# aous72/OpenJPH

Hardware: AMD Instinct MI355X
Metric: Msamples/s encode+decode, 8K 12-bit 4:4:4; achieved HBM GB/s vs roofline (higher is better)
Workload: dtype f32; 1 GPU; c3_8k_444_12b_irv97; width=7680, height=4320, components=3, bit_depth=12, wavelet=9/7 irreversible, decomps=5, hip_streams=1, sample_container_bits=16, roundtrip_max_abs_err=8

## Files before the change

openjph_amd/csrc/kernels_ht_enc.hip:

```cpp
#include <hip/hip_runtime.h>
#include <stdint.h>
#include <cstdlib>
#include <type_traits>
#include "../../include/ojphgpu.h"
#include "ht_quant.h"
#include "ht_tables.h"

namespace ojphgpu {
__device__ __attribute__((aligned(16))) uint16_t g_enc_vlc[2][2048];
}

namespace {

using ojphgpu::to_sign_mag;

constexpr int MS_WORDS = 512;
constexpr int VLC_WORDS = 64;
constexpr int MEL_CAP = 192;
constexpr int VLC_CAP = 3072 - MEL_CAP;
constexpr int WAVES = 4;
constexpr uint32_t NARROW_MAX_W = 64;

constexpr int MS_WORDS64 = 1040;
constexpr int VLC_WORDS64 = 96;
// ... 198 lines not shown
    for (int i = 0; i < 6; ++i) {
      V t = (active && !first_row) ? sample(x0 - 1 + i, y0 - 1) : (V)0;
      V v = ((V)(t + t) >> p) & ~(V)1;
      Eab[i] = expo(v); Sab[i] = v != 0;
    }

    uint32_t rho[2], cq[2], uq[2], Uq[2], tup[2];
    V msv[8]; uint32_t msl[8];
    uint32_t rho_q[2] = { 0, 0 }, emax[2] = { 0, 0 }, e[8];
#pragma unroll
    for (int i = 0; i < 8; ++i) {
      e[i] = expo(val[i]);
      if (val[i]) rho_q[i >> 2] |= 1u << (i & 3);
      emax[i >> 2] = max(emax[i >> 2], e[i]);
    }
    if (!has_q1) { rho_q[1] = 0; emax[1] = 0; }
    uint32_t rho_prev = __shfl_up(rho_q[1], 1);
    if (lane == 0) rho_prev = carry_rho;
    if (px == 0) rho_prev = 0;
    carry_rho = rdlane(rho_q[1], 63);
#pragma unroll
    for (int q = 0; q < 2; ++q) {
      const uint32_t rl = q == 0 ? rho_prev : rho_q[0];
      uint32_t kappa = 1, c;
      if (first_row) c = (rl >> 1) | (rl & 1);
      else {
        const uint32_t* E = Eab + 2 * q; const uint32_t* S = Sab + 2 * q;
        uint32_t me = max(max(E[0], E[1]), max(E[2], E[3]));
        int max_e = (int)me - 1;
        if (rho_q[q] & (rho_q[q] - 1)) kappa = (uint32_t)max(1, max_e);
        c = (S[0] | S[1]) | ((S[2] | S[3]) << 2) | ((rl & 4) >> 1) | ((rl & 8) >> 2);
      }
      const uint32_t U = max(emax[q], kappa), u = U - kappa;
      uint32_t eps = 0;
      if (u > 0) {
#pragma unroll
        for (int nn = 0; nn < 4; ++nn) eps |= (uint32_t)(e[q * 4 + nn] == emax[q]) << nn;
      }
      const uint32_t tuple = s_vlc[first_row ? 0 : 1][(c << 8) + (rho_q[q] << 4) + eps];
      rho[q] = rho_q[q]; cq[q] = c; uq[q] = u; Uq[q] = U; tup[q] = tuple;
#pragma unroll
      for (int nn = 0; nn < 4; ++nn) {
        const int i = q * 4 + nn;
        const uint32_t m = ((rho_q[q] >> nn) & 1u) ? U - ((tuple >> nn) & 1u) : 0u;
        const V s = val[i] ? val[i] - 2u + sgn[i] : (V)0;
        msl[i] = m;
        msv[i] = m ? (s & ((m >= VBITS ? (V)0 : ((V)1 << m)) - (V)1)) : (V)0;
      }
    }
    const bool q0on = active, q1on = has_q1;
    if (!q1on) { uq[1] = 0; for (int nn = 4; nn < 8; ++nn) { msl[nn] = 0; msv[nn] = 0; } }
    if (!q0on) { uq[0] = 0; for (int nn = 0; nn < 4; ++nn) { msl[nn] = 0; msv[nn] = 0; } }
    any_sig |= (__ballot(((rho[0] | rho[1]) != 0 && active) || over != 0u) != 0ull) ? 1u : 0u;

    uint64_t vb = 0; uint32_t vl = 0;
    auto vadd = [&](uint32_t c, uint32_t len) { vb |= (uint64_t)c << vl; vl += len; };
    uint32_t x0e = 0, xl0 = 0, x1e = 0, xl1 = 0;
    auto uvlc = [](uint32_t u, uint32_t& pre, uint32_t& pl, uint32_t& suf, uint32_t& sl, uint32_t& ext, uint32_t& el) {
      ext = 0; el = 0;
      if (u == 0) { pre = 0; pl = 0; suf = 0; sl = 0; }
      else if (u == 1) { pre = 1; pl = 1; suf = 0; sl = 0; }
      else if (u == 2) { pre = 2; pl = 2; suf = 0; sl = 0; }
      else if (u <= 4) { pre = 4; pl = 3; suf = u - 3; sl = 1; }
      else if (u <= 32 || !S64) { pre = 0; pl = 3; suf = u - 5; sl = 5; }
      else { pre = 0; pl = 3; suf = 28u + ((u - 33u) & 3u); sl = 5; ext = (u - 33u) >> 2; el = 4; }
    };
    bool ev2_valid = false; uint32_t ev2_bit = 0;
    if (q0on) {
      vadd(tup[0] >> 8, (tup[0] >> 4) & 7);
      if (q1on) vadd(tup[1] >> 8, (tup[1] >> 4) & 7);
      const uint32_t u0 = uq[0], u1 = uq[1];
      uint32_t p0, l0, s0, sl0, p1, l1, s1, sl1;
      if (first_row && u0 > 0 && u1 > 0) { ev2_valid = true; ev2_bit = min(u0, u1) > 2; }
      if (first_row && u0 > 2 && u1 > 2) {
        uvlc(u0 - 2, p0, l0, s0, sl0, x0e, xl0); uvlc(u1 - 2, p1, l1, s1, sl1, x1e, xl1);
        vadd(p0, l0); vadd(p1, l1); vadd(s0, sl0); vadd(s1, sl1); vadd(x0e, xl0); vadd(x1e, xl1);
      } else if (first_row && u0 > 2 && u1 > 0) {
        uvlc(u0, p0, l0, s0, sl0, x0e, xl0);
        vadd(p0, l0); vadd(u1 - 1, 1); vadd(s0, sl0); vadd(x0e, xl0);
      } else {
        uvlc(u0, p0, l0, s0, sl0, x0e, xl0); uvlc(u1, p1, l1, s1, sl1, x1e, xl1);
        vadd(p0, l0); vadd(p1, l1); vadd(s0, sl0); vadd(s1, sl1); vadd(x0e, xl0); vadd(x1e, xl1);
      }
    }

    const bool ev0_valid = q0on && cq[0] == 0, ev1_valid = q1on && cq[1] == 0;
    const uint32_t ev0_bit = rho[0] != 0, ev1_bit = rho[1] != 0;
    {
      const uint32_t cnt = (uint32_t)ev0_valid + (uint32_t)ev1_valid + (uint32_t)ev2_valid;
      const uint32_t incl = wave_incl_scan(cnt, lane);
      const uint32_t nev = rdlane(incl, 63);
      uint32_t at = incl - cnt;
      if (ev0_valid) { if (ev0_bit) atomicOr(&L.ev[at >> 5], 1u << (at & 31)); at++; }
      if (ev1_valid) { if (ev1_bit) atomicOr(&L.ev[at >> 5], 1u << (at & 31)); at++; }
      if (ev2_valid) { if (ev2_bit) atomicOr(&L.ev[at >> 5], 1u << (at & 31)); at++; }
      wave_sync();
      uint32_t done = 0;
      while (done < nev) {
        const uint32_t w = done >> 5, sh = done & 31;
        uint32_t word = rdfirst(L.ev[w]) >> sh;
        const uint32_t avail = min(32u - sh, nev - done);
        if (word == 0) { mel_zero_run(mel, L.mel, avail, lane); done += avail; continue; }
        const uint32_t z = (uint32_t)__builtin_ctz(word);
        if (z >= avail) { mel_zero_run(mel, L.mel, avail, lane); done += avail; continue; }
        mel_zero_run(mel, L.mel, z, lane);
        mel_one(mel, L.mel, lane);
        done += z + 1;
      }
      wave_sync();
      if (lane < 8) L.ev[lane] = 0;
    }

    {
      uint32_t tot = 0;
#pragma unroll
      for (int i = 0; i < 8; ++i) tot += msl[i];
      const uint32_t incl = wave_incl_scan(tot, lane);
      const uint32_t T = ms_carry + rdlane(incl, 63);
      uint32_t at = ms_carry + incl - tot;
#pragma unroll
      for (int i = 0; i < 8; ++i) {
        if constexpr (S64) {
          const uint32_t lo = msl[i] < 32u ? msl[i] : 32u;
          or_bits(L.ms, at, (uint32_t)msv[i], lo);
          if (msl[i] > 32u) or_bits(L.ms, at + 32u, (uint32_t)(msv[i] >> 32), msl[i] - 32u);
        } else or_bits(L.ms, at, (uint32_t)msv[i], msl[i]);
        at += msl[i];
      }
      wave_sync();
      uint32_t pos = 0;
      for (;;) {
        const uint32_t first_n = ms_ff ? 7u : 8u;
        const uint32_t start = pos + (lane == 0 ? 0u : first_n + 8u * (uint32_t)(lane - 1));
        const uint32_t nb = lane == 0 ? first_n : 8u;
        const bool ok = start + nb <= T;
        const uint32_t v = ok ? get_bits(L.ms, start, nb) : 0u;
        const uint64_t m_ok = __ballot(ok), m_ff = __ballot(ok && v == 0xFF);
        const uint32_t n_ok = m_ok == ~0ull ? 64u : (uint32_t)__builtin_ctzll(~m_ok);
        const uint32_t f_ff = m_ff ? (uint32_t)__builtin_ctzll(m_ff) : 64u;
        const uint32_t nc = min(n_ok, f_ff + 1u);
        if (nc == 0) break;
        if (ms_k + nc > ms_cap) { err = 1; break; }
        if ((uint32_t)lane < nc) ms_out[ms_k + lane] = (uint8_t)v;
        ms_k += nc;
        pos += first_n + 8u * (nc - 1u);
        ms_ff = f_ff < n_ok ? 1u : 0u;
      }
      const uint32_t rem = T - pos;
      const uint32_t cv = rem ? get_bits(L.ms, pos, rem) : 0u;
      wave_sync();
      const uint32_t used = (T >> 5) + 2;
      for (uint32_t i = lane; i < used && i < (uint32_t)MSW; i += 64) L.ms[i] = 0;
      wave_sync();
      if (lane == 0) L.ms[0] = cv;
      ms_carry = rem;
      wave_sync();
    }

    {
      const uint32_t incl = wave_incl_scan(vl, lane);
      const uint32_t T = v_carry + rdlane(incl, 63);
      {
        const uint32_t at = v_carry + incl - vl, lo = vl < 32u ? vl : 32u;
        or_bits(L.vlc, at, (uint32_t)vb, lo);
        if (vl > 32u) or_bits(L.vlc, at + 32u, (uint32_t)(vb >> 32), vl - 32u);
      }
      wave_sync();
      uint32_t pos = 0;
      for (;;) {
        const uint32_t start = pos + 8u * (uint32_t)lane;
        const bool have7 = start + 7 <= T, have8 = start + 8 <= T;
        const uint32_t v8 = have7 ? get_bits(L.vlc, start, 8) : 0u;
        uint32_t pv = __shfl_up(v8, 1);
        if (lane == 0) pv = v_prev;
        const bool special = have7 && pv > 0x8F && (v8 & 0x7F) == 0x7F;
        const bool stop = !have8 && !special;
        const uint64_t m_sp = __ballot(special), m_st = __ballot(stop);
        const uint32_t fs = m_sp ? (uint32_t)__builtin_ctzll(m_sp) : 64u;
        const uint32_t ft = m_st ? (uint32_t)__builtin_ctzll(m_st) : 64u;
        const uint32_t n8 = min(fs, ft);
        const bool sp = fs < ft;
        if (n8 == 0 && !sp) break;
        if (v_pos + n8 + 1 >= (uint32_t)VLC_CAP) { err = 1; break; }
        if ((uint32_t)lane < n8) *(vlc_last - (v_pos + lane)) = (uint8_t)v8;
        if (sp && (uint32_t)lane == fs) *(vlc_last - (v_pos + lane)) = 0x7F;
        const uint32_t last8 = n8 ? rdlane(v8, (int)(n8 - 1)) : v_prev;
        v_pos += n8 + (sp ? 1u : 0u);
        pos += 8u * n8 + (sp ? 7u : 0u);
        v_prev = sp ? 0x7Fu : last8;
      }
      const uint32_t rem = T - pos;
      const uint32_t cv = rem ? get_bits(L.vlc, pos, rem) : 0u;
      wave_sync();
      for (int i = lane; i < VLW; i += 64) L.vlc[i] = 0;
      wave_sync();
      if (lane == 0) L.vlc[0] = cv;
      v_carry = rem;
      wave_sync();
    }
    if (err) break;
  }

  err |= mel.err;
  uint32_t total = 0, ms_len = ms_k;
  if (!err && any_sig) {
    const uint32_t ms_tmp0 = rdfirst(L.ms[0]);
    if (ms_carry) {
      const uint32_t maxb = ms_ff ? 7u : 8u, t = maxb - ms_carry;
      const uint32_t tmp = ms_tmp0 | ((0xFFu & ((1u << t) - 1u)) << ms_carry);
      if (tmp != 0xFF) {
        if (ms_len >= ms_cap) err = 1;
        else { if (lane == 0) ms_out[ms_len] = (uint8_t)tmp; ms_len++; }
      }
    } else if (ms_ff) ms_len--;
    if (mel.run > 0) mel_put(mel, L.mel, 1, 1, lane);
    const uint32_t need = mel.lastff ? 7u : 8u, remaining = need - mel.nb;
    const uint32_t mel_tmp = (mel.acc << remaining) & 0xFFu;
    const uint32_t mel_mask = (0xFFu << remaining) & 0xFFu;
    const uint32_t vlc_tmp = rdfirst(L.vlc[0]) & 0xFFu;
    const uint32_t vlc_mask = v_carry ? (0xFFu >> (8 - v_carry)) : 0u;
    if ((mel_mask | vlc_mask) != 0) {
      if (mel.pos >= (uint32_t)MEL_CAP) err = 1;
      else {
        const uint32_t fuse = mel_tmp | vlc_tmp;
        if (((((fuse ^ mel_tmp) & mel_mask) | ((fuse ^ vlc_tmp) & vlc_mask)) == 0) && fuse != 0xFF && v_pos > 1) {
          if (lane == 0) L.mel[mel.pos] = (uint8_t)fuse;
          mel.pos++;
        } else {
          if (v_pos >= (uint32_t)VLC_CAP) err = 1;
          else {
            if (lane == 0) { L.mel[mel.pos] = (uint8_t)mel_tmp; *(vlc_last - v_pos) = (uint8_t)vlc_tmp; }
            mel.pos++; v_pos++;
          }
        }
      }
    }
    err |= mel.err;
    total = ms_len + mel.pos + v_pos;
  }
  wave_sync();
  __threadfence_block();

  uint32_t off = 0;
  if (err) total = 0;
  if (total) {
    off = claim_output(cursor, regions, nreg, bi, (total + 3u) & ~3u, out_cap, lane);
    if (off == 0xFFFFFFFFu) { err = 1; total = 0; off = 0; }
  }
  if (total) {
    const uint32_t scup = mel.pos + v_pos;
    uint8_t* dst = out + off;
    const uint8_t* vsrc = vlc_last - v_pos + 1;
    for (uint32_t i = lane; i < total; i += 64) {
      uint32_t b;
      if (i < ms_len) b = ms_out[i];
      else if (i < ms_len + mel.pos) b = L.mel[i - ms_len];
      else b = vsrc[i - ms_len - mel.pos];
      if (i == total - 1) b = scup >> 4;
      else if (i == total - 2) b = (b & 0xF0u) | (scup & 0xFu);
      dst[i] = (uint8_t)b;
    }
  }
  if (lane == 0) {
    results[bi].offset = off; results[bi].length = total;
    if (err) atomicOr(status, 1u);
  }
}

#ifndef ABL
#define ABL 0
#endif
#ifndef NWAVES
#define NWAVES 4
#endif
#ifndef NOUT_CAP
#define NOUT_CAP 5120
#endif
#ifndef NWAVES_PER_EU
#define NWAVES_PER_EU 4
#endif
constexpr uint32_t OUT_CAP = NOUT_CAP;
constexpr int PMS_WORDS = 576;
constexpr int PVLC_WORDS = 112;

struct NarrowLds {
  uint32_t out[OUT_CAP / 4];
  uint32_t ms[PMS_WORDS];
  uint32_t vlc[PVLC_WORDS];
  uint8_t  mel[MEL_CAP + 8];
};
static_assert(MEL_CAP + 8 >= 4 * (MEL_CAP / 4 + 2), "raw MEL words");
#ifndef NWG_PER_CU
#define NWG_PER_CU 4
#endif
static_assert(NWG_PER_CU * (2 * 2048 * 2 + 64 * 4 + NWAVES * sizeof(NarrowLds)) <= 160 * 1024, "the narrow kernel's workgroups do not fit the LDS as planned");

#ifndef ENC_ROWS_W4V
#define ENC_ROWS_W4V 1
#endif
#ifndef ENC_ROWS_AHEAD
#define ENC_ROWS_AHEAD 1
#endif
static_assert(ENC_ROWS_AHEAD == 1 || ENC_ROWS_AHEAD == 2, "one or two steps of rows in flight");

struct __attribute__((aligned(4))) U4 { uint32_t x, y, z, w; };
typedef uint32_t U4V __attribute__((ext_vector_type(4), aligned(4)));

template <int KIND> struct RawRows {
  uint32_t t[4], b[4];
  __device__ __forceinline__ void arrived() { asm volatile("" : "+v"(t[0]), "+v"(t[1]), "+v"(t[2]), "+v"(t[3]), "+v"(b[0]), "+v"(b[1]), "+v"(b[2]), "+v"(b[3])); }
  __device__ __forceinline__ uint32_t top(int k) const { return t[k]; }
  __device__ __forceinline__ uint32_t bot(int k) const { return b[k]; }
};
template <> struct RawRows<1> {
  U4V t, b;
  __device__ __forceinline__ void arrived() { asm volatile("" : "+v"(t), "+v"(b)); }
  __device__ __forceinline__ uint32_t top(int k) const { return t[k]; }
  __device__ __forceinline__ uint32_t bot(int k) const { return b[k]; }
};

__device__ __forceinline__ uint32_t dpp_prev(uint32_t v) { return (uint32_t)__builtin_amdgcn_update_dpp(0, (int)v, 0x138, 0xF, 0xF, false); }
__device__ __forceinline__ uint32_t dpp_next(uint32_t v) { return (uint32_t)__builtin_amdgcn_update_dpp(0, (int)v, 0x130, 0xF, 0xF, false); }

__device__ __forceinline__ uint32_t uvlc_word(uint32_t u)
{
  const uint32_t lo = u < 3u ? 1u : 0u, mid = (u >= 3u && u < 5u) ? 1u : 0u;
  const uint32_t pre = lo ? u : (mid ? 4u : 0u);
  const uint32_t pl = u < 3u ? u : 3u;
  const uint32_t suf = lo ? 0u : (mid ? u - 3u : u - 5u);
  const uint32_t sl = lo ? 0u : (mid ? 1u : 5u);
  return pre | (pl << 8) | (suf << 16) | (sl << 24);
}

constexpr uint64_t MEL_PM = (1ull << 0) | (1ull << 1) | (1ull << 2) | (1ull << 3) | (1ull << 5) | (1ull << 7) | (1ull << 9) | (1ull << 13) |
                            (1ull << 17) | (1ull << 21) | (1ull << 29) | (1ull << 37) | (1ull << 53);
constexpr uint32_t MEL_RAW_BITS = 8u * MEL_CAP;
constexpr uint32_t MEL_RAW_WORDS = MEL_CAP / 4 + 2;

__device__ __forceinline__ void mel_at(uint32_t k, uint32_t c, uint32_t& K, uint32_t& run, uint32_t& ones, uint32_t& pKm1)
{
  const uint32_t full = c >= 85u ? (c - 53u) >> 5 : 0u;
  const uint32_t cc = c - 32u * full;
  if (cc >= 53u) { K = 12u; run = cc - 53u; pKm1 = 37u; }
  else {
    const uint64_t m = MEL_PM << (63u - cc);
    const uint32_t lz = (uint32_t)__builtin_clzll(m);
    K = (uint32_t)__popcll(m) - 1u; run = lz;
    const uint64_t m2 = m & ~(0x8000000000000000ull >> lz);
    pKm1 = m2 ? cc - (uint32_t)__builtin_clzll(m2) : 0u;
  }
  ones = K - k + full;
}

__device__ __forceinline__ void mel_stuff(const uint32_t* raw, uint32_t total_bits, uint8_t* out, MelState& st, int lane)
{
  uint32_t pos = 0, bytes = 0, lastff = 0, err = 0;
  for (;;) {
    const uint32_t first = lastff ? 7u : 8u;
    const uint32_t start = pos + (lane == 0 ? 0u : first + 8u * ((uint32_t)lane - 1u));
    const uint32_t len = lane == 0 ? first : 8u;
    const bool have = start + len <= total_bits;
    const uint32_t w = start >> 5, sh = start & 31u;
    const uint32_t x = have ? __funnelshift_l(raw[w + 1], raw[w], sh) >> (32u - len) : 0u;
    const uint64_t m_have = __ballot(have), m_ff = __ballot(have && x == 0xFFu);
    const uint32_t n_ok = m_have == ~0ull ? 64u : (uint32_t)__builtin_ctzll(~m_have);
    const uint32_t f_ff = m_ff ? (uint32_t)__builtin_ctzll(m_ff) : 64u;
    const uint32_t nc = min(n_ok, f_ff + 1u);
    if (nc == 0) break;
    if (bytes + nc > (uint32_t)MEL_CAP) { err = 1; break; }
    if ((uint32_t)lane < nc) out[bytes + lane] = (uint8_t)x;
    bytes += nc;
    pos += first + 8u * (nc - 1u);
    lastff = f_ff < n_ok ? 1u : 0u;
  }
  const uint32_t left = total_bits - pos;
  const uint32_t w = pos >> 5, sh = pos & 31u;
  const uint32_t x = left ? rdfirst(__funnelshift_l(raw[w + 1], raw[w], sh)) >> (32u - left) : 0u;
  st.k = 0; st.run = 0; st.acc = x; st.nb = left; st.pos = bytes; st.lastff = lastff; st.err = err;
}

template <bool REV, int LOGP>
__global__ __launch_bounds__(64 * NWAVES) __attribute__((amdgpu_waves_per_eu(NWAVES_PER_EU, 8))) void ht_encode_kernel(
    const ojphgpu_cb_desc* __restrict__ blocks, uint32_t n, const uint32_t* __restrict__ coef,
    uint8_t* __restrict__ scratch, uint8_t* __restrict__ out, uint32_t out_cap,
    ojphgpu_cb_result* __restrict__ results, uint32_t* __restrict__ cursor, uint32_t* __restrict__ status,
    const uint32_t* __restrict__ regions, uint32_t nreg)
{
  __shared__ __attribute__((aligned(16))) uint16_t s_vlc[2][2048];
  __shared__ uint32_t s_uvlc[64];
  __shared__ NarrowLds s_wave[NWAVES];
  const int lane = threadIdx.x & 63;
  const int wave = __builtin_amdgcn_readfirstlane((int)(threadIdx.x >> 6));
  const uint32_t bi = blockIdx.x * NWAVES + wave;
  struct DescWords { uint32_t v[sizeof(ojphgpu_cb_desc) / 4]; } dw;
  __builtin_memcpy(&dw, blocks + min(bi, n - 1u), sizeof dw);
  ojphgpu_cb_desc d;
  __builtin_memcpy(&d, &dw, sizeof d);
  static_assert(offsetof(ojphgpu_cb_desc, K_max) == 16 && offsetof(ojphgpu_cb_desc, reversible) == 17, "K_max, reversible: bytes 0, 1 of dword 4");
  uint32_t kr = dw.v[4];
  asm volatile("" : "+s"(kr));
  const uint32_t d_K_max = kr & 0xFFu, d_reversible = (kr >> 8) & 0xFFu;
  const uint32_t W = d.w, H = d.h;
  constexpr uint32_t PPR = 1u << LOGP, RPS = 64u >> LOGP;
  const bool my_width = LOGP == 5 ? (W > NARROW_MAX_W && W <= 4u * PPR) : (W <= NARROW_MAX_W && W <= 4u * PPR);
  const bool my_kind = bi < n && my_width && ((d_reversible & 1u) != 0) == REV && (d_reversible & 4u) == 0;
  const bool mine = my_kind && W != 0 && H != 0;
  NarrowLds& L = s_wave[wave];
  uint8_t* outb = reinterpret_cast<uint8_t*>(L.out);
  const uint32_t K = d_K_max, p = 31u - K;
  constexpr bool rev = REV;
  const float delta_inv = rev ? 0.0f : __fdiv_rn(1.0f, d.delta);
  const uint32_t* src = coef + d.coef_off;
  const uint32_t pitch = d.pitch;
  uint8_t* ms_spill = scratch + d.data_off;
  const uint32_t ms_cap = d.scratch_cap > (uint32_t)VLC_CAP ? d.scratch_cap - VLC_CAP : 0;
  const uint32_t QW = (W + 1) >> 1, QH = (H + 1) >> 1, PW = (QW + 1) >> 1;
  const uint32_t nsteps = (QH + RPS - 1u) / RPS;

  const uint32_t r = (uint32_t)lane >> LOGP, px = (uint32_t)lane & (PPR - 1u);
  const bool pxok = px < PW;
  const uint32_t x0 = 4u * px;
  const bool has_q1 = pxok && x0 + 2 < W;

  auto prologue = [&](bool clear) __attribute__((always_inline)) {
    for (int i = threadIdx.x; i < 2 * 2048 / 8; i += blockDim.x)
      reinterpret_cast<uint4*>(&s_vlc[0][0])[i] = reinterpret_cast<const uint4*>(&ojphgpu::g_enc_vlc[0][0])[i];
    if (threadIdx.x < 64) s_uvlc[threadIdx.x] = uvlc_word(threadIdx.x);
    if (clear) {
      for (int i = lane; i < PMS_WORDS; i += 64) L.ms[i] = 0;
      for (int i = lane; i < PVLC_WORDS; i += 64) L.vlc[i] = 0;
      if (lane < (int)MEL_RAW_WORDS) reinterpret_cast<uint32_t*>(L.mel)[lane] = 0;
      wave_sync();
      if (lane == 0) { L.vlc[0] = 0xF; outb[OUT_CAP - 1] = 0xFF; }
      wave_sync();
    }
    __syncthreads();
  };
  if (!mine) {
    prologue(false);
    if (my_kind && lane == 0) { results[bi].offset = 0; results[bi].length = 0; }
    return;
  }
  const bool w4 = (W & 3u) == 0;

  uint32_t ms_pend = 0, ms_base = 0, ms_k = 0, ms_ff = 0;
  uint32_t v_pend = 4, v_base = 0, v_pos = 1, v_prev = 0xFF;
  uint32_t mel_k = 0, mel_c = 0, mel_bits = 0, mel_err = 0;
  uint32_t* const mel_raw = reinterpret_cast<uint32_t*>(L.mel);
  auto mel_or = [&](uint32_t code, uint32_t len, uint32_t pos) __attribute__((always_inline)) {
    if (len) {
      const uint32_t sh = pos & 31u, w = pos >> 5;
      const uint64_t v = (uint64_t)code << (64u - sh - len);
      atomicOr(&mel_raw[w], (uint32_t)(v >> 32));
      if (sh + len > 32u) atomicOr(&mel_raw[w + 1u], (uint32_t)v);
    }
  };
  auto mel_ones = [&](uint32_t n) __attribute__((always_inline)) {
    if (n == 0u) return;
    if (mel_bits + n > MEL_RAW_BITS) mel_err = 1;
    else if (lane == 0) mel_or((1u << n) - 1u, n, mel_bits);
    mel_bits += n;
  };
  auto mel_zeros = [&](uint32_t n) __attribute__((always_inline)) {
    mel_c += n;
    if (mel_c >= 85u) {
      const uint32_t full = (mel_c - 53u) >> 5;
      mel_ones(12u - mel_k + full);
      mel_k = 12u; mel_c -= 32u * full;
    }
  };
  uint32_t err = 0, any_sig = 0;
  bool prev_sig = false;

  uint32_t ms_out = 0;
  auto flush_stage = [&]() __attribute__((always_inline)) -> bool {
    const uint32_t have = ms_k - ms_out, nwd = have >> 2;
    if (ms_out + 4u * nwd > ms_cap) return false;
    uint32_t* g = reinterpret_cast<uint32_t*>(ms_spill + ms_out);
    for (uint32_t i = lane; i < nwd; i += 64) g[i] = L.out[i];
    const uint32_t keep = L.out[nwd];
    wave_sync();
    if (lane == 0) L.out[0] = keep;
    wave_sync();
    ms_out += 4u * nwd;
    return true;
  };

  uint32_t last_S = 0;

  auto ms_windows = [&](uint32_t base, uint32_t T, bool flush) __attribute__((always_inline)) -> uint32_t {
    uint32_t pos = base;
    for (;;) {
      const uint32_t first_n = ms_ff ? 7u : 8u;
      if (!flush && pos + first_n + 8u * 255u > T) break;
      const uint32_t start = pos + (lane == 0 ? 0u : first_n + 8u * (4u * (uint32_t)lane - 1u));
      const uint32_t lead = lane == 0 ? first_n : 8u;
      uint32_t v = 0, cnt = 0;
      if (start + lead <= T) {
        const uint32_t w = start >> 5, sh = start & 31u;
        v = __funnelshift_r(L.ms[w], L.ms[w + 1], sh);
        cnt = min(4u, 1u + ((T - start - lead) >> 3));
      }
      const uint32_t bytes = (lane == 0 && first_n == 7u) ? ((v & 0x7Fu) | ((v >> 7) << 8)) : v;
      const uint32_t have = cnt == 4u ? 0xFFFFFFFFu : (1u << (8u * cnt)) - 1u;
      const uint32_t ffm = (((bytes & 0x7F7F7F7Fu) + 0x01010101u) & bytes & 0x80808080u) & have;
      const uint64_t m_full = __ballot(cnt == 4u), m_ff = __ballot(ffm != 0u);
      const uint32_t nfull = m_full == ~0ull ? 64u : (uint32_t)__builtin_ctzll(~m_full);
      const uint32_t n_ok = nfull == 64u ? 256u : 4u * nfull + rdlane(cnt, (int)nfull);
      uint32_t f_ff = 256u;
      if (m_ff) { const uint32_t lf = (uint32_t)__builtin_ctzll(m_ff); f_ff = 4u * lf + ((uint32_t)__builtin_ctz(rdlane(ffm, (int)lf)) >> 3); }
      const uint32_t nc = min(n_ok, f_ff + 1u);
      if (nc == 0) break;
      if (ms_k - ms_out + nc + v_pos + 72u > OUT_CAP && !flush_stage()) { err = 1; break; }
      uint8_t* dstb = outb + (ms_k - ms_out) + 4u * (uint32_t)lane;
      const uint32_t mine = nc > 4u * (uint32_t)lane ? min(4u, nc - 4u * (uint32_t)lane) : 0u;
      if (mine > 0) dstb[0] = (uint8_t)bytes;
      if (mine > 1) dstb[1] = (uint8_t)(bytes >> 8);
      if (mine > 2) dstb[2] = (uint8_t)(bytes >> 16);
      if (mine > 3) dstb[3] = (uint8_t)(bytes >> 24);
      ms_k += nc;
      pos += first_n + 8u * (nc - 1u);
      ms_ff = f_ff < n_ok ? 1u : 0u;
    }
    return pos;
  };
  auto ms_windows_full = [&](uint32_t base, uint32_t T) __attribute__((always_inline)) -> uint32_t {
    uint32_t pos = base;
    for (;;) {
      const uint32_t first_n = ms_ff ? 7u : 8u;
      if (pos + first_n + 8u * 255u > T) break;
      const uint32_t start = lane == 0 ? pos : pos + first_n - 8u + 32u * (uint32_t)lane;
      const uint32_t w = start >> 5, sh = start & 31u;
      uint32_t bytes = __funnelshift_r(L.ms[w], L.ms[w + 1], sh);
      if (ms_ff) bytes = lane == 0 ? ((bytes & 0x7Fu) | ((bytes >> 7) << 8)) : bytes;
      const uint32_t ffm = ((bytes & 0x7F7F7F7Fu) + 0x01010101u) & bytes & 0x80808080u;
      const uint64_t m_ff = __ballot(ffm != 0u);
      uint32_t nc = 256u, ff = 0u;
      if (m_ff) { const uint32_t lf = (uint32_t)__builtin_ctzll(m_ff); nc = 4u * lf + ((uint32_t)__builtin_ctz(rdlane(ffm, (int)lf)) >> 3) + 1u; ff = 1u; }
      if (ms_k - ms_out + nc + v_pos + 72u > OUT_CAP && !flush_stage()) { err = 1; break; }
      if (4u * (uint32_t)lane < nc) __builtin_memcpy(outb + (ms_k - ms_out) + 4u * (uint32_t)lane, &bytes, 4);
      ms_k += nc;
      pos += first_n + 8u * (nc - 1u);
      ms_ff = ff;
    }
    return pos;
  };
  auto vlc_windows_full = [&](uint32_t base, uint32_t T) __attribute__((always_inline)) -> uint32_t {
    uint32_t pos = base;
    for (;;) {
      if (pos + 8u * 64u > T) break;
      const uint32_t v8 = get_bits(L.vlc, pos + 8u * (uint32_t)lane, 8);
      uint32_t pv = dpp_prev(v8);
      if (lane == 0) pv = v_prev;
      const uint64_t m_sp = __ballot(pv > 0x8Fu && (v8 & 0x7Fu) == 0x7Fu);
      uint32_t n8 = 64u, sp = 0u;
      if (m_sp) { n8 = (uint32_t)__builtin_ctzll(m_sp); sp = 1u; }
      if (v_pos + n8 + 1 >= (uint32_t)VLC_CAP) { err = 1; break; }
      if (ms_k - ms_out + v_pos + n8 + 72u > OUT_CAP && !flush_stage()) { err = 1; break; }
      if ((uint32_t)lane < n8 + sp) outb[OUT_CAP - 1 - (v_pos + lane)] = (uint8_t)((uint32_t)lane == n8 ? 0x7Fu : v8);
      const uint32_t last8 = n8 ? rdlane(v8, (int)(n8 - 1)) : v_prev;
      v_pos += n8 + sp;
      pos += 8u * n8 + 7u * sp;
      v_prev = sp ? 0x7Fu : last8;
    }
    return pos;
  };
  auto vlc_windows = [&](uint32_t base, uint32_t T, bool flush) __attribute__((always_inline)) -> uint32_t {
    uint32_t pos = base;
    for (;;) {
      if (!flush && pos + 8u * 64u > T) break;
      const uint32_t start = pos + 8u * (uint32_t)lane;
      const bool have7 = start + 7 <= T, have8 = start + 8 <= T;
      const uint32_t v8 = have7 ? get_bits(L.vlc, start, 8) : 0u;
      uint32_t pv = dpp_prev(v8);
      if (lane == 0) pv = v_prev;
      const bool special = have7 && pv > 0x8F && (v8 & 0x7F) == 0x7F;
      const bool stop = !have8 && !special;
      const uint64_t m_sp = __ballot(special), m_st = __ballot(stop);
      const uint32_t fs = m_sp ? (uint32_t)__builtin_ctzll(m_sp) : 64u;
      const uint32_t ft = m_st ? (uint32_t)__builtin_ctzll(m_st) : 64u;
      const uint32_t n8 = min(fs, ft);
      const bool sp = fs < ft;
      if (n8 == 0 && !sp) break;
      if (v_pos + n8 + 1 >= (uint32_t)VLC_CAP) { err = 1; break; }
      if (ms_k - ms_out + v_pos + n8 + 72u > OUT_CAP && !flush_stage()) { err = 1; break; }
      if ((uint32_t)lane < n8) outb[OUT_CAP - 1 - (v_pos + lane)] = (uint8_t)v8;
      if (sp && (uint32_t)lane == fs) outb[OUT_CAP - 1 - (v_pos + lane)] = 0x7F;
      const uint32_t last8 = n8 ? rdlane(v8, (int)(n8 - 1)) : v_prev;
      v_pos += n8 + (sp ? 1u : 0u);
      pos += 8u * n8 + (sp ? 7u : 0u);
      v_prev = sp ? 0x7Fu : last8;
    }
    return pos;
  };
  auto compact = [&](uint32_t* buf, uint32_t pos, uint32_t T, uint32_t nwords) __attribute__((always_inline)) -> uint32_t {
    const uint32_t rem = T - pos, nw = (rem + 31u) >> 5;
    const uint32_t w0 = pos >> 5, sh = pos & 31u;
    uint32_t keep = 0;
    if ((uint32_t)lane < nw) {
      keep = __funnelshift_r(buf[w0 + lane], buf[w0 + lane + 1], sh);
      if (lane == (int)nw - 1 && (rem & 31u)) keep &= (1u << (rem & 31u)) - 1u;
    }
    wave_sync();
    const uint32_t used = min((T >> 5) + 2u, nwords);
    for (uint32_t i = lane; i < used; i += 64) buf[i] = 0;
    wave_sync();
    if ((uint32_t)lane < nw) buf[lane] = keep;
    wave_sync();
    return rem;
  };

  auto or32 = [&](uint32_t* buf, uint32_t pos, uint32_t v) __attribute__((always_inline)) {
    const uint32_t sh = pos & 31u;
    uint32_t* wp = buf + (pos >> 5);
    atomicOr(wp, v << sh);
    atomicOr(wp + 1, (v >> 1) >> (sh ^ 31u));
  };
  auto nz_flags = [](uint32_t x) __attribute__((always_inline)) -> uint32_t { return (x + 0x7F7F7F7Fu) & 0x80808080u; };
  auto gather4 = [](uint32_t f) __attribute__((always_inline)) -> uint32_t { return ((f >> 7) * 0x10204080u) >> 28; };
  typedef unsigned short us2 __attribute__((ext_vector_type(2)));
  auto pk_max = [](uint32_t a, uint32_t b2) __attribute__((always_inline)) -> uint32_t {
    return __builtin_bit_cast(uint32_t, __builtin_elementwise_max(__builtin_bit_cast(us2, a), __builtin_bit_cast(us2, b2)));
  };
  auto left_of = [&](uint32_t v) __attribute__((always_inline)) -> uint32_t {
    if (LOGP == 4) return (uint32_t)__builtin_amdgcn_update_dpp(0, (int)v, 0x111, 0xF, 0xF, false);
    const uint32_t t = dpp_prev(v); return px == 0 ? 0u : t;
  };
  auto right_of = [&](uint32_t v) __attribute__((always_inline)) -> uint32_t {
    if (LOGP == 4) return (uint32_t)__builtin_amdgcn_update_dpp(0, (int)v, 0x101, 0xF, 0xF, false);
    const uint32_t t = dpp_next(v); return px == PPR - 1u ? 0u : t;
  };

  auto code_steps = [&](auto kind_c) __attribute__((always_inline)) {
    constexpr int KIND = decltype(kind_c)::value;
    using Rows = RawRows<KIND>;
    auto load_rows = [&](uint32_t qy, Rows& R) __attribute__((always_inline)) {
      const uint32_t qyc = min(qy, QH - 1u);
      const uint32_t y0 = 2u * qyc, y1 = min(y0 + 1u, H - 1u);
      const uint32_t* r0 = src + (size_t)y0 * pitch;
      const uint32_t* r1 = src + (size_t)y1 * pitch;
      if (ABL & 32) { r0 = coef + (size_t)bi * 4096u + y0 * 64u; r1 = coef + (size_t)bi * 4096u + y1 * 64u; }
      if constexpr (KIND == 1) {
        const uint32_t xc = min(x0, W - 4u);
        R.t = *reinterpret_cast<const U4V*>(r0 + xc);
        R.b = *reinterpret_cast<const U4V*>(r1 + xc);
      } else if (KIND == 0 && w4) {
        const uint32_t xc = min(x0, W - 4u);
        const U4 a = *reinterpret_cast<const U4*>(r0 + xc);
        const U4 c = *reinterpret_cast<const U4*>(r1 + xc);
        R.t[0] = a.x; R.t[1] = a.y; R.t[2] = a.z; R.t[3] = a.w;
        R.b[0] = c.x; R.b[1] = c.y; R.b[2] = c.z; R.b[3] = c.w;
      } else {
#pragma unroll
        for (int k = 0; k < 4; ++k) { const uint32_t xk = min(x0 + (uint32_t)k, W - 1u); R.t[k] = r0[xk]; R.b[k] = r1[xk]; }
      }
    };
    Rows A;
    [[maybe_unused]] Rows B;
    load_rows(r, A);
    if constexpr (ENC_ROWS_AHEAD == 2) load_rows(r + RPS, B);
    prologue(true);

    float colf[4]; uint32_t colm[4];
#pragma unroll
    for (int k = 0; k < 4; ++k) {
      const bool in = pxok && x0 + (uint32_t)k < W;
      colf[k] = in ? ldexpf(delta_inv, -(int)p) : 0.0f;
      colm[k] = in ? (1u << (31u - p)) - 1u : 0u;
    }
    const bool ragged = (QH & (RPS - 1u)) != 0 || (H & 1u) != 0;

    auto one_step = [&](const uint32_t step, Rows& R) __attribute__((always_inline)) {
      const uint32_t qy = RPS * step + r;
      const bool active = pxok && qy < QH;
      R.arrived();
      uint32_t rt[4], rb[4];
#pragma unroll
      for (int k = 0; k < 4; ++k) { rt[k] = R.top(k); rb[k] = R.bot(k); }
      if (ragged && step + 1 == nsteps) {
        const bool bot = active && 2u * qy + 1u < H;
#pragma unroll
        for (int k = 0; k < 4; ++k) { rt[k] = active ? rt[k] : 0u; rb[k] = bot ? rb[k] : 0u; }
      }
      uint32_t mu[8], sx[8];
      uint32_t nz = 0;
#pragma unroll
      for (int k = 0; k < 4; ++k) {
#pragma unroll
        for (int j = 0; j < 2; ++j) {
          const uint32_t raw = j ? rb[k] : rt[k];
          if (rev) {
            const int v = (int)raw;
            const uint32_t a = (uint32_t)(v >= 0 ? v : -v);
            mu[2 * k + j] = a & colm[k];
            sx[2 * k + j] = raw | (a << p);
            nz |= a;
          } else {
            mu[2 * k + j] = (uint32_t)__fmul_rn(fabsf(__uint_as_float(raw)), colf[k]);
            sx[2 * k + j] = raw;
            nz |= mu[2 * k + j];
          }
        }
      }
      if (__ballot((nz >> K) != 0u) != 0ull) {
        any_sig |= (rev ? __ballot(((nz >> K) & 1u) != 0u) != 0ull : true) ? 1u : 0u;
        if (!rev) {
          nz = 0;
#pragma unroll
          for (int i = 0; i < 8; ++i) { mu[i] = (mu[i] >> K) ? 0u : mu[i]; nz |= mu[i]; }
        }
      }
      if (rev) nz &= (1u << K) - 1u;
      if (ENC_ROWS_AHEAD == 2 || step + 1 < nsteps) load_rows(qy + ENC_ROWS_AHEAD * RPS, R);
      if (ENC_ROWS_AHEAD == 2 && err) return;
      if (ABL & 16) { any_sig |= (uint32_t)(__ballot((mu[0] ^ mu[1] ^ mu[2] ^ mu[3] ^ mu[4] ^ mu[5] ^ mu[6] ^ mu[7]) == 0x12345u) != 0ull); return; }
      {
        const bool step_sig = __ballot(nz != 0u) != 0ull;
        const bool skip = !step_sig && !prev_sig;
        prev_sig = step_sig;
        if (skip) {
          const uint32_t nq = (uint32_t)__popcll(__ballot(active)) + (uint32_t)__popcll(__ballot(has_q1 && active));
          mel_zeros(nq);
          last_S = 0;
          return;
        }
        any_sig |= step_sig ? 1u : 0u;
      }
      uint32_t e[8], sv[8];
#pragma unroll
      for (int i = 0; i < 8; ++i) {
        const uint32_t m1 = mu[i] - 1u, w = m1 + mu[i];
        e[i] = (0u - (uint32_t)__builtin_clz(w)) & 31u;
        sv[i] = __builtin_amdgcn_alignbit(m1, sx[i], 31);
      }
      const uint32_t ep0 = e[0] | (e[1] << 8) | (e[2] << 16) | (e[3] << 24);
      const uint32_t ep1 = e[4] | (e[5] << 8) | (e[6] << 16) | (e[7] << 24);
      const uint32_t sf0 = nz_flags(ep0), sf1 = nz_flags(ep1);
      const uint32_t rho0 = gather4(sf0), rho1 = gather4(sf1);
      const uint32_t emax0 = max(max(e[0], e[1]), max(e[2], e[3])), emax1 = max(max(e[4], e[5]), max(e[6], e[7]));

      uint32_t S;
      {
        const uint32_t b0 = e[1], b1 = e[3], b2 = e[5], b3 = e[7];
        const uint32_t m12 = max(b1, b2);
        const uint32_t own = max(b0, m12) | (max(m12, b3) << 16);
        const uint32_t X = b3 | (b0 << 16), Y = b0 | (b3 << 16);
        const uint32_t nb = (left_of(X) & 0xFFFFu) | (right_of(X) & 0xFFFF0000u);
        const uint32_t mx = pk_max(own, nb);
        const uint32_t F = (pk_max(nb, Y) + 0x007F001Fu) & 0x00800020u;
        const uint32_t f12 = ((m12 + 31u) & 32u) * 0x10004u;
        S = mx | F | f12;
      }
      const uint32_t give = (uint32_t)lane >= 64u - PPR ? last_S : S;
      const uint32_t above = (uint32_t)__builtin_amdgcn_ds_bpermute((int)(((lane - (int)PPR) & 63) << 2), (int)give);
      last_S = S;

      const uint32_t rho_left = left_of(rho1);
      uint32_t uq[2], tup[2], Uq[2], chi[2];
#pragma unroll
      for (int q = 0; q < 2; ++q) {
        const uint32_t rl = q == 0 ? rho_left : rho0, rho = q ? rho1 : rho0, emax = q ? emax1 : emax0, ep = q ? ep1 : ep0;
        const uint32_t aq = q ? above >> 16 : above;
        uint32_t c5 = (aq & 0xA0u) | ((4u * rl + 48u) & 64u);
        uint32_t tsel = 2048u;
        if (step == 0) {
          const bool fr = qy == 0;
          c5 = fr ? ((rl >> 1) | (rl & 1u)) << 5 : c5;
          tsel = fr ? 0u : 2048u;
        }
        const uint32_t multi = 0u - ((0xFEE8u >> rho) & 1u);
        const uint32_t me = aq & 31u;
        const uint32_t kappa = 1u + ((me > 2u ? me - 2u : 0u) & multi);
        const uint32_t U = max(emax, kappa), u = U - kappa;
        const uint32_t xe = ep ^ (emax * 0x01010101u);
        uint32_t eps = gather4((nz_flags(xe) ^ 0x80808080u));
        eps = u ? eps : 0u;
        tup[q] = (&s_vlc[0][0])[tsel + (c5 << 3) + (rho << 4) + eps];
        uq[q] = u; Uq[q] = U; chi[q] = c5;
      }

      uint32_t vb = 0, vl = 0;
      bool ev2_valid = false; uint32_t ev2_bit = 0;
      {
        const uint32_t u0 = uq[0], u1 = has_q1 ? uq[1] : 0u;
        vb = tup[0] >> 8; vl = (tup[0] >> 4) & 7u;
        if (has_q1) { vb |= (tup[1] >> 8) << vl; vl += (tup[1] >> 4) & 7u; }
        const bool first_row = qy == 0;
        const bool both_big = first_row && u0 > 2 && u1 > 2;
        const bool one_big = first_row && !both_big && u0 > 2 && u1 > 0;
        ev2_valid = first_row && u0 > 0 && u1 > 0; ev2_bit = min(u0, u1) > 2;
        const uint32_t w0 = s_uvlc[both_big ? u0 - 2u : u0];
        uint32_t w1 = s_uvlc[both_big ? u1 - 2u : u1];
        if (one_big) w1 = (u1 - 1u) | (1u << 8);
        vb |= (w0 & 0xFFu) << vl; vl += (w0 >> 8) & 0xFFu;
        vb |= (w1 & 0xFFu) << vl; vl += (w1 >> 8) & 0xFFu;
        vb |= ((w0 >> 16) & 0xFFu) << vl; vl += w0 >> 24;
        vb |= ((w1 >> 16) & 0xFFu) << vl; vl += w1 >> 24;
        if (!active) { vb = 0; vl = 0; ev2_valid = false; }
      }

      uint32_t mp[2];
#pragma unroll
      for (int q = 0; q < 2; ++q) {
        const uint32_t sf = q ? sf1 : sf0;
        const uint32_t sig = (sf - (sf >> 7)) | sf;
        const uint32_t ek = ((tup[q] & 15u) * 0x204081u) & 0x01010101u;
        mp[q] = (Uq[q] * 0x01010101u - ek) & sig;
      }
      const uint32_t tot0 = __builtin_amdgcn_sad_u8(mp[0], 0u, 0u), tot = __builtin_amdgcn_sad_u8(mp[1], 0u, tot0);

      const uint32_t incl = wave_incl_scan(tot | (vl << 16), lane);
      const uint32_t sums = rdlane(incl, 63);
      const uint32_t step_bits = sums & 0xFFFFu, step_vbits = sums >> 16;
      if (ms_base + ms_pend + step_bits + 64u > 32u * (uint32_t)PMS_WORDS) {
        ms_pend = compact(L.ms, ms_base, ms_base + ms_pend, PMS_WORDS);
        ms_base = 0;
      }
      if (v_base + v_pend + step_vbits + 64u > 32u * (uint32_t)PVLC_WORDS) {
        v_pend = compact(L.vlc, v_base, v_base + v_pend, PVLC_WORDS);
        v_base = 0;
      }

      if (ABL & 8) { any_sig |= (uint32_t)(__ballot((vb ^ mp[0] ^ mp[1] ^ sv[0] ^ sv[7] ^ chi[1] ^ incl) == 0x12345u) != 0ull); return; }
      if (!(ABL & 1)) {
        const uint32_t fl = ((active && chi[0] == 0u) ? (rho0 != 0u ? 0x11u : 0x01u) : 0u) |
                            ((active && has_q1 && chi[1] == 0u) ? (rho1 != 0u ? 0x22u : 0x02u) : 0u) |
                            ((step == 0 && ev2_valid) ? (ev2_bit != 0u ? 0x44u : 0x04u) : 0u);
        if (__ballot((fl & 7u) != 0u) != 0ull) {
          const uint32_t nwords = step == 0 ? 3u : 2u;
          for (uint32_t wd = 0; wd < nwords; ++wd) {
            const uint32_t e = 64u * wd + (uint32_t)lane;
            uint32_t from, slot;
            if (step == 0) {
              const uint32_t e2 = e - 3u * PPR;
              const bool fr = e < 3u * PPR;
              from = fr ? e / 3u : PPR + (e2 >> 1);
              slot = fr ? e - 3u * (e / 3u) : e2 & 1u;
            } else { from = e >> 1; slot = e & 1u; }
            const uint32_t g = (uint32_t)__builtin_amdgcn_ds_bpermute((int)((from & 63u) << 2), (int)fl) >> slot;
            const bool valid = from < 64u && (g & 1u) != 0u, one = valid && (g & 16u) != 0u;
            const uint64_t Vw = __ballot(valid), Bw = __ballot(one);
            if (Vw == 0ull) continue;
            const uint32_t nvalid = (uint32_t)__popcll(Vw);
            if (Bw == 0ull) { mel_c += nvalid; continue; }
            const uint32_t before = __builtin_amdgcn_mbcnt_hi((uint32_t)(Vw >> 32), __builtin_amdgcn_mbcnt_lo((uint32_t)Vw, 0u));
            uint32_t info = 0;
            uint32_t consumed = 0;
            {
              uint64_t ones = Bw;
              while (ones) {
                const uint32_t l = (uint32_t)__builtin_ctzll(ones);
                asm("s_bitset0_b64 %0, %1" : "+s"(ones) : "s"(l));
                const uint32_t bf = rdlane(before, (int)l);
                mel_c += bf - consumed; consumed = bf + 1u;
                info = (uint32_t)lane == l ? (mel_k | (mel_c << 4)) : info;
                uint32_t K, pKm1;
                if (mel_c >= 85u) mel_c -= (mel_c - 53u) & ~31u;
                if (mel_c >= 53u) { K = 12u; pKm1 = 37u; }
                else {
                  const uint64_t m = MEL_PM << (63u - mel_c);
                  K = (uint32_t)__popcll(m) - 1u;
                  const uint64_t m2 = m & ~(0x8000000000000000ull >> (uint32_t)__builtin_clzll(m));
                  pKm1 = m2 ? mel_c - (uint32_t)__builtin_clzll(m2) : 0u;
                }
                int km1 = (int)K - 1;
                asm("s_max_i32 %0, %1, 0" : "=s"(km1) : "s"(km1) : "scc");
                mel_k = (uint32_t)km1; mel_c = pKm1;
              }
            }
            uint32_t code = 0, len = 0;
            if (one) {
              uint32_t K, run, nones, pKm1;
              mel_at(info & 15u, info >> 4, K, run, nones, pKm1);
              const uint32_t eb = mel_exp(K);
              code = (((1u << nones) - 1u) << (eb + 1u)) | run;
              len = nones + eb + 1u;
            }
            const uint32_t at_incl = wave_incl_scan(len, lane);
            const uint32_t wbits = rdlane(at_incl, 63);
            if (mel_bits + wbits > MEL_RAW_BITS) mel_err = 1;
            else mel_or(code, len, mel_bits + at_incl - len);
            mel_bits += wbits;
            mel_c += nvalid - consumed;
          }
          mel_zeros(0u);
        }
      }

      if (ABL & 2) { any_sig |= (uint32_t)(__ballot((vb ^ mp[0] ^ mp[1] ^ sv[0] ^ sv[3] ^ sv[5] ^ sv[7] ^ incl) == 0x12345u) != 0ull); }
      else {
        const uint32_t at = ms_base + ms_pend + (incl & 0xFFFFu) - tot;
        const bool wide_bits = __ballot(max(Uq[0], Uq[1]) > 16u) != 0ull;
        if (!wide_bits) {
          uint32_t pr[4], ln[2];
#pragma unroll
          for (int q = 0; q < 2; ++q) {
            const uint32_t m = mp[q];
// ... 231 lines not shown
```

Baseline: 105,300 Msamples/s.

## Resolve VLC bit-stuffing across a whole wave window with iterative ballot passes

```diff
diff --git a/openjph_amd/csrc/kernels_ht_enc.hip b/openjph_amd/csrc/kernels_ht_enc.hip
--- a/openjph_amd/csrc/kernels_ht_enc.hip
+++ b/openjph_amd/csrc/kernels_ht_enc.hip
@@ -524,6 +524,16 @@
 #define ENC_ROWS_AHEAD 1
 #endif
 static_assert(ENC_ROWS_AHEAD == 1 || ENC_ROWS_AHEAD == 2, "one or two steps of rows in flight");
+#ifndef ENC_STUFF_WHOLE
+#define ENC_STUFF_WHOLE 2
+#endif
+#ifndef ENC_VLC_LANE_BYTES
+#define ENC_VLC_LANE_BYTES 2
+#endif
+#ifndef ENC_STUFF_MAX
+#define ENC_STUFF_MAX 7
+#endif
+static_assert(ENC_STUFF_MAX >= 1 && 1 + 4 * ENC_STUFF_MAX <= 31, "a lane's bytes move down by at most 31 bits (one funnel shift over two lanes' words)");
 
 struct __attribute__((aligned(4))) U4 { uint32_t x, y, z, w; };
 typedef uint32_t U4V __attribute__((ext_vector_type(4), aligned(4)));
@@ -710,6 +720,87 @@
 
   uint32_t last_S = 0;
 
+#if ENC_STUFF_WHOLE & 1
+  auto ms_resolve = [&](uint32_t n, uint32_t& y, uint32_t& k, uint32_t& p7, uint32_t& nl, uint32_t& used, uint32_t& ff) __attribute__((always_inline)) {
+    const uint32_t prev = dpp_prev(n);
+    k = lane ? ms_ff : 0u; p7 = lane ? 0u : ms_ff;
+    uint32_t tot = ms_ff, f_last = 64u, b3_last = 0u;
+    uint64_t open = ~0ull;
+    nl = 64u;
+    for (uint32_t it = 0;; ++it) {
+      uint32_t x = __funnelshift_l(prev, n, k);
+      x = p7 ? x + (x & 0xFFFFFF80u) : x;
+      x = (x & 0xFFu) == 0xFFu ? x + (x & 0xFFFF8000u) : x;
+      x = (x & 0xFF00u) == 0xFF00u ? x + (x & 0xFF800000u) : x;
+      x = (x & 0xFF0000u) == 0xFF0000u ? x & 0x7FFFFFFFu : x;
+      y = x;
+      const uint32_t ffm = ((x & 0x7F7F7F7Fu) + 0x01010101u) & x & 0x80808080u;
+      const uint64_t m = __ballot(ffm != 0u) & open;
+      if (!m) break;
+      const uint32_t f = (uint32_t)__builtin_ctzll(m);
+      if (it == (uint32_t)ENC_STUFF_MAX) { nl = f; break; }
+      const uint32_t g = rdlane(ffm, (int)f), c = (uint32_t)__popc(g & 0x00808080u), b3 = g >> 31;
+      k += ((uint32_t)lane > f ? c : 0u) + ((uint32_t)lane > f + 1u ? b3 : 0u);
+      p7 = (uint32_t)lane == f + 1u ? b3 : p7;
+      tot += c + b3;
+      open = ~1ull << f;
+      f_last = f; b3_last = b3;
+    }
+    ff = f_last + 1u == nl ? b3_last : 0u;
+    used = 32u * nl - tot + ff;
+  };
+  auto ms_windows = [&](uint32_t base, uint32_t T, bool flush) __attribute__((always_inline)) -> uint32_t {
+    uint32_t pos = base;
+    for (;;) {
+      const uint32_t first_n = ms_ff ? 7u : 8u;
+      if (!flush && pos + first_n + 8u * 255u > T) break;
+      const uint32_t start = pos + 32u * (uint32_t)lane;
+      uint32_t n = 0;
+      if (start < T) n = __funnelshift_r(L.ms[start >> 5], L.ms[(start >> 5) + 1u], start & 31u);
+      uint32_t y, k, p7, nl, used, ff;
+      ms_resolve(n, y, k, p7, nl, used, ff);
+      const uint32_t e0 = start - k + (p7 ? 7u : 8u);
+      const uint32_t e1 = e0 + ((y & 0xFFu) == 0xFFu ? 7u : 8u);
+      const uint32_t e2 = e1 + ((y & 0xFF00u) == 0xFF00u ? 7u : 8u);
+      const uint32_t e3 = e2 + ((y & 0xFF0000u) == 0xFF0000u ? 7u : 8u);
+      uint32_t cnt = (e0 <= T ? 1u : 0u) + (e1 <= T ? 1u : 0u) + (e2 <= T ? 1u : 0u) + (e3 <= T ? 1u : 0u);
+      if ((uint32_t)lane >= nl) cnt = 0;
+      const uint32_t e_last = cnt == 4u ? e3 : (cnt == 3u ? e2 : (cnt == 2u ? e1 : e0));
+      const uint64_t m_full = __ballot(cnt == 4u);
+      const uint32_t nfull = m_full == ~0ull ? 64u : (uint32_t)__builtin_ctzll(~m_full);
+      const uint32_t nc = nfull == 64u ? 256u : 4u * nfull + rdlane(cnt, (int)nfull);
+      if (nc == 0) break;
+      if (ms_k - ms_out + nc + v_pos + 72u > OUT_CAP && !flush_stage()) { err = 1; break; }
+      uint8_t* dstb = outb + (ms_k - ms_out) + 4u * (uint32_t)lane;
+      const uint32_t mine = nc > 4u * (uint32_t)lane ? min(4u, nc - 4u * (uint32_t)lane) : 0u;
+      if (mine > 0) dstb[0] = (uint8_t)y;
+      if (mine > 1) dstb[1] = (uint8_t)(y >> 8);
+      if (mine > 2) dstb[2] = (uint8_t)(y >> 16);
+      if (mine > 3) dstb[3] = (uint8_t)(y >> 24);
+      const uint32_t ll = (nc - 1u) >> 2;
+      ms_k += nc;
+      pos = rdlane(e_last, (int)ll);
+      ms_ff = ((rdlane(y, (int)ll) >> (8u * ((nc - 1u) & 3u))) & 0xFFu) == 0xFFu ? 1u : 0u;
+    }
+    return pos;
+  };
+  auto ms_windows_full = [&](uint32_t base, uint32_t T) __attribute__((always_inline)) -> uint32_t {
+    uint32_t pos = base;
+    for (;;) {
+      if (pos + (ms_ff ? 7u : 8u) + 8u * 255u > T) break;
+      const uint32_t start = pos + 32u * (uint32_t)lane;
+      const uint32_t n = __funnelshift_r(L.ms[start >> 5], L.ms[(start >> 5) + 1u], start & 31u);
+      uint32_t y, k, p7, nl, used, ff;
+      ms_resolve(n, y, k, p7, nl, used, ff);
+      if (ms_k - ms_out + 4u * nl + v_pos + 72u > OUT_CAP && !flush_stage()) { err = 1; break; }
+      if ((uint32_t)lane < nl) __builtin_memcpy(outb + (ms_k - ms_out) + 4u * (uint32_t)lane, &y, 4);
+      ms_k += 4u * nl;
+      pos += used;
+      ms_ff = ff;
+    }
+    return pos;
+  };
+#else
   auto ms_windows = [&](uint32_t base, uint32_t T, bool flush) __attribute__((always_inline)) -> uint32_t {
     uint32_t pos = base;
     for (;;) {
@@ -767,6 +858,91 @@
     }
     return pos;
   };
+#endif
+#if ENC_STUFF_WHOLE & 2
+  constexpr uint32_t VB = ENC_VLC_LANE_BYTES;
+  static_assert(VB == 1 || VB == 2, "one or two VLC bytes per lane");
+  static_assert(ENC_STUFF_MAX <= 8 && 8 * 127 + 8 * 240 + 64 <= 32 * PVLC_WORDS, "the shift a lane's load allows for; pending bytes plus a step");
+  auto vlc_resolve = [&](uint32_t q, uint32_t back, uint32_t& o, uint32_t& k, uint32_t& p0, uint32_t& s1, uint32_t& nl, uint32_t& used) __attribute__((always_inline)) {
+    k = 0u; p0 = 0u; nl = 64u;
+    uint64_t open = ~0ull;
+    uint32_t it = 0;
+    for (;; ++it) {
+      const uint32_t x = q >> (back - k);
+      const uint32_t b0 = x & 0xFFu, o0 = p0 ? 0x7Fu : b0;
+      uint32_t last = o0;
+      s1 = 0u;
+      if (VB == 2) {
+        const uint32_t b1 = (p0 ? x >> 7 : x >> 8) & 0xFFu;
+        s1 = (o0 > 0x8Fu && (b1 & 0x7Fu) == 0x7Fu) ? 1u : 0u;
+        last = s1 ? 0x7Fu : b1;
+      }
+      o = VB == 2 ? o0 | (last << 8) : o0;
+      uint32_t pv = dpp_prev(last);
+      if (lane == 0) pv = v_prev;
+      const bool s0 = !p0 && pv > 0x8Fu && (b0 & 0x7Fu) == 0x7Fu;
+      const uint64_t m = __ballot(s0 || s1 != 0u) & open;
+      if (!m) break;
+      const uint32_t f = (uint32_t)__builtin_ctzll(m);
+      if (it == (uint32_t)ENC_STUFF_MAX) { nl = f; break; }
+      p0 = ((uint32_t)lane == f && s0) ? 1u : p0;
+      k += (uint32_t)lane > f ? 1u : 0u;
+      open = ~1ull << f;
+    }
+    used = 8u * VB * nl - it;
+  };
+  auto vlc_windows = [&](uint32_t base, uint32_t T, bool flush) __attribute__((always_inline)) -> uint32_t {
+    uint32_t pos = base;
+    for (;;) {
+      if (!flush && pos + 8u * VB * 64u > T) break;
+      const uint32_t nominal = 8u * VB * (uint32_t)lane, back = min(nominal, 8u);
+      const uint32_t org = pos + nominal - back;
+      uint32_t q = 0;
+      if (org < T) q = __funnelshift_r(L.vlc[org >> 5], L.vlc[(org >> 5) + 1u], org & 31u);
+      uint32_t o, k, p0, s1, nl, used;
+      vlc_resolve(q, back, o, k, p0, s1, nl, used);
+      const uint32_t e0 = pos + nominal - k + (p0 ? 7u : 8u), e1 = e0 + (s1 ? 7u : 8u);
+      uint32_t cnt = (e0 <= T ? 1u : 0u) + ((VB == 2 && e1 <= T) ? 1u : 0u);
+      if ((uint32_t)lane >= nl) cnt = 0;
+      const uint32_t e_last = cnt == 2u ? e1 : e0;
+      const uint64_t m_full = __ballot(cnt == VB);
+      const uint32_t nfull = m_full == ~0ull ? 64u : (uint32_t)__builtin_ctzll(~m_full);
+      const uint32_t nc = nfull == 64u ? 64u * VB : VB * nfull + rdlane(cnt, (int)nfull);
+      if (nc == 0) break;
+      if (v_pos + nc + 1 >= (uint32_t)VLC_CAP) { err = 1; break; }
+      if (ms_k - ms_out + v_pos + nc + 72u > OUT_CAP && !flush_stage()) { err = 1; break; }
+      if (VB * (uint32_t)lane < nc) outb[OUT_CAP - 1 - (v_pos + VB * lane)] = (uint8_t)o;
+      if (VB == 2 && 2u * (uint32_t)lane + 1u < nc) outb[OUT_CAP - 2 - (v_pos + 2 * lane)] = (uint8_t)(o >> 8);
+      const uint32_t ll = (nc - 1u) / VB;
+      v_pos += nc;
+      pos = rdlane(e_last, (int)ll);
+      v_prev = (rdlane(o, (int)ll) >> (8u * ((nc - 1u) & (VB - 1u)))) & 0xFFu;
+    }
+    return pos;
+  };
+  auto vlc_windows_full = [&](uint32_t base, uint32_t T) __attribute__((always_inline)) -> uint32_t {
+    uint32_t pos = base;
+    for (;;) {
+      if (pos + 8u * VB * 64u > T) break;
+      const uint32_t nominal = 8u * VB * (uint32_t)lane, back = min(nominal, 8u);
+      const uint32_t org = pos + nominal - back;
+      const uint32_t q = __funnelshift_r(L.vlc[org >> 5], L.vlc[(org >> 5) + 1u], org & 31u);
+      uint32_t o, k, p0, s1, nl, used;
+      vlc_resolve(q, back, o, k, p0, s1, nl, used);
+      const uint32_t nc = VB * nl;
+      if (v_pos + nc + 1 >= (uint32_t)VLC_CAP) { err = 1; break; }
+      if (ms_k - ms_out + v_pos + nc + 72u > OUT_CAP && !flush_stage()) { err = 1; break; }
+      if ((uint32_t)lane < nl) {
+        if (VB == 2) { const uint16_t two = (uint16_t)((o >> 8) | (o << 8)); __builtin_memcpy(outb + OUT_CAP - 2 - (v_pos + 2 * lane), &two, 2); }
+        else outb[OUT_CAP - 1 - (v_pos + lane)] = (uint8_t)o;
+      }
+      v_pos += nc;
+      pos += used;
+      v_prev = (rdlane(o, (int)(nl - 1u)) >> (8u * (VB - 1u))) & 0xFFu;
+    }
+    return pos;
+  };
+#else
   auto vlc_windows_full = [&](uint32_t base, uint32_t T) __attribute__((always_inline)) -> uint32_t {
     uint32_t pos = base;
     for (;;) {
@@ -815,6 +991,7 @@
     }
     return pos;
   };
+#endif
   auto compact = [&](uint32_t* buf, uint32_t pos, uint32_t T, uint32_t nwords) __attribute__((always_inline)) -> uint32_t {
     const uint32_t rem = T - pos, nw = (rem + 31u) >> 5;
     const uint32_t w0 = pos >> 5, sh = pos & 31u;
```

After: 105,100 Msamples/s. No clear change (-0.2%).
